# GreatV/oar-ocr

Hardware: AMD Instinct MI355X
Metric: images/sec end-to-end PP-OCRv6 det+rec (higher is better)
Workload: dtype f32; 1 GPU; PP-OCRv6-tiny-class det+rec (synthetic-weight graphs: det 447089 params, rec 1135700 params, V=6906), batch=32 synthetic 960x960 pages per GPU, 40 text lines/page; timed region = u8 pages in pageable HOST memory -> oar_ocr_predict -> oar_ocr_decode -> sorted boxes + texts + scores on the host; image_batch_size=32, region_batch_size=256, parallelism=image-parallel x1

## Files before the change

oar_ocr_amd/csrc/kernels.hip:

```cpp
#include "kernels.h"

#include <hip/hip_ext.h>
#include <hip/hip_runtime.h>

#include <algorithm>
#include <cstdlib>
#include <type_traits>

#include "common.h"
#include "kernels_dev.h"

namespace oar {
namespace k {

template <int K, int SH, int S, int TW, int TH, bool GAP = false>
__global__ __launch_bounds__(256) void conv_dw_tiled_kernel(ConvP p) {
    extern __shared__ float4 dw_w[];
    const int C4 = p.Cout >> 2;
    for (int i = threadIdx.x; i < K * K * C4; i += blockDim.x) dw_w[i] = reinterpret_cast<const float4*>(p.w)[i];
    __syncthreads();
    const int wtiles = (p.Wo + TW - 1) / TW, htiles = (p.Ho + TH - 1) / TH;
    const long total = (long)p.N * htiles * wtiles * C4;
    constexpr int NCOL = (TW - 1) * S + K, NROW = (TH - 1) * SH + K;
    const long per_xcd = (total + 7) / 8;
// ... 139 lines not shown
#define DW2(KV, SHV, SWV, THV)                                                                                                                              \
    do {                                                                                                                                                    \
        if (lds > 64 * 1024) {                                                                                                                              \
            OAR_MAX_LDS_ONCE((conv_dw_tiled_kernel<KV, SHV, SWV, TW, THV>), 96 * 1024);                    \
        }                                                                                                                                                   \
        hipExtLaunchKernelGGL((conv_dw_tiled_kernel<KV, SHV, SWV, TW, THV>), g, b, lds, s, ps.start(), ps.stop(), 0, p);                                    \
    } while (0)
#define DW2G(KV, SHV, SWV, THV)                                                                                                                             \
    do {                                                                                                                                                    \
        if (lds > 64 * 1024) {                                                                                                                              \
            OAR_MAX_LDS_ONCE((conv_dw_tiled_kernel<KV, SHV, SWV, TW, THV, true>), 96 * 1024);                    \
        }                                                                                                                                                   \
        hipExtLaunchKernelGGL((conv_dw_tiled_kernel<KV, SHV, SWV, TW, THV, true>), g, b, lds, s, ps.start(), ps.stop(), 0, p);                              \
    } while (0)
#define DWG(KV, SHV, SWV)                                  \
    do {                                                   \
        if (TH == 2) DW2G(KV, SHV, SWV, 2);                \
        else DW2G(KV, SHV, SWV, 1);                        \
    } while (0)
#define DW(KV, SHV, SWV)                                   \
    do {                                                   \
        if (TH == 2) DW2(KV, SHV, SWV, 2);                 \
        else DW2(KV, SHV, SWV, 1);                         \
    } while (0)
    if (p.gap_part) {
        if (p.sh == 1 && p.sw == 1) DWG(5, 1, 1);
        else if (p.sh == 2 && p.sw == 2) DWG(5, 2, 2);
        else if (p.sh == 2 && p.sw == 1) DWG(5, 2, 1);
        else DWG(5, 1, 2);
    } else
    if (fits && sq && p.kh == 3 && p.sh == 1 && p.sw == 1) DW(3, 1, 1);
    else if (fits && sq && p.kh == 3 && p.sh == 2 && p.sw == 2) DW(3, 2, 2);
    else if (fits && sq && p.kh == 3 && p.sh == 2 && p.sw == 1) DW(3, 2, 1);
    else if (fits && sq && p.kh == 3 && p.sh == 1 && p.sw == 2) DW(3, 1, 2);
    else if (fits && sq && p.kh == 5 && p.sh == 1 && p.sw == 1) DW(5, 1, 1);
    else if (fits && sq && p.kh == 5 && p.sh == 2 && p.sw == 2) DW(5, 2, 2);
    else if (fits && sq && p.kh == 5 && p.sh == 2 && p.sw == 1) DW(5, 2, 1);
    else if (fits && sq && p.kh == 5 && p.sh == 1 && p.sw == 2) DW(5, 1, 2);
    else hipExtLaunchKernelGGL(conv_dw_kernel, dim3(grid_for(total)), b, 0, s, ps.start(), ps.stop(), 0, p);
#undef DW2
#undef DW
#undef DW2G
#undef DWG
}

__global__ __launch_bounds__(256) void conv_smallcin_kernel(ConvP p) {
    __shared__ float ws[128 * 16];
    const int K = p.kh * p.kw * p.Cin;
    const int co0 = blockIdx.y * 16;
    for (int i = threadIdx.x; i < K * 16; i += 256) {
        int k = i >> 4, c = i & 15;
        ws[i] = (co0 + c < p.Cout) ? p.w[(long)k * p.Cout + co0 + c] : 0.f;
    }
    __syncthreads();
    const long total = (long)p.N * p.Ho * p.Wo;
    for (long pix = (long)blockIdx.x * blockDim.x + threadIdx.x; pix < total; pix += (long)gridDim.x * blockDim.x) {
        int ow = (int)(pix % p.Wo); long t = pix / p.Wo;
        int oh = (int)(t % p.Ho); long n = t / p.Ho;
        float acc[16];
#pragma unroll
        for (int c = 0; c < 16; ++c) acc[c] = (p.bias && co0 + c < p.Cout) ? p.bias[co0 + c] : 0.f;
        const float* xb = p.x + n * (long)p.H * p.W * p.Cin;
        for (int a = 0; a < p.kh; ++a) {
            int ih = oh * p.sh - p.pt + a * p.dh;
            if (ih < 0 || ih >= p.H) continue;
            for (int b = 0; b < p.kw; ++b) {
                int iw = ow * p.sw - p.pl + b * p.dw;
                if (iw < 0 || iw >= p.W) continue;
                const float* xp = xb + ((long)ih * p.W + iw) * p.Cin;
                const float* wp = ws + (a * p.kw + b) * p.Cin * 16;
                for (int ci = 0; ci < p.Cin; ++ci) {
                    float xv = xp[ci];
#pragma unroll
                    for (int c = 0; c < 16; ++c) acc[c] = fmaf(xv, wp[ci * 16 + c], acc[c]);
                }
            }
        }
        float* o = p.y + pix * p.y_ld + co0;
        const bool vec = (co0 + 16 <= p.Cout) && ((p.y_ld & 3) == 0);
#pragma unroll
        for (int c = 0; c < 16; ++c) {
            if (p.residual && co0 + c < p.Cout) acc[c] += p.residual[pix * p.y_ld + co0 + c];
            acc[c] = apply_act(acc[c], p.act.kind, p.act.alpha, p.act.beta);
        }
        if (vec) {
#pragma unroll
            for (int q = 0; q < 4; ++q) *reinterpret_cast<float4*>(o + q * 4) = make_float4(acc[q * 4], acc[q * 4 + 1], acc[q * 4 + 2], acc[q * 4 + 3]);
        } else {
            for (int c = 0; c < 16 && co0 + c < p.Cout; ++c) o[c] = acc[c];
        }
    }
}

typedef const __attribute__((address_space(4))) float sfloat;
template <bool CRNN, bool K3, bool SW>
__global__ __launch_bounds__(256) void conv_smallcin_u8_kernel(ConvP p, StemU8 st) {
    __shared__ float ws[SW ? 1 : 128 * 16];
    __shared__ float lut[CRNN ? 256 : 1];
    __shared__ float ot[4 * 64 * 17];
    const int K = p.kh * p.kw * 3;
    const int co0 = blockIdx.y * 16;
    if (!SW)
        for (int i = threadIdx.x; i < K * 16; i += 256) {
            int k = i >> 4, c = i & 15;
            ws[i] = (co0 + c < p.Cout) ? p.w[(long)k * p.Cout + co0 + c] : 0.f;
        }
    sfloat* wsc = (sfloat*)(uintptr_t)(p.w + co0);
    if (CRNN) lut[threadIdx.x] = ((float)threadIdx.x / 255.0f - 0.5f) / 0.5f;
    __syncthreads();
    const long per_image = (long)p.Ho * p.Wo;
    const float a0 = st.alpha[0], a1 = st.alpha[1], a2 = st.alpha[2], b0 = st.beta[0], b1 = st.beta[1], b2 = st.beta[2];
    const int s0 = st.src[0], s1 = st.src[1], s2 = st.src[2];
    const int n = blockIdx.z;
    const uint8_t* __restrict__ pg = CRNN ? st.dev[n].ptr : st.pages[n];
    const int img_w = CRNN ? st.dev[n].w : p.W;
    for (long pix = (long)blockIdx.x * blockDim.x + threadIdx.x; pix - (threadIdx.x & 63) < per_image; pix += (long)gridDim.x * blockDim.x) {
        const bool live = pix < per_image;
        const long pixc = live ? pix : per_image - 1;
        const int ow = (int)(pixc % p.Wo), oh = (int)(pixc / p.Wo);
        float acc[16];
#pragma unroll
        for (int c = 0; c < 16; ++c) acc[c] = (p.bias && co0 + c < p.Cout) ? p.bias[co0 + c] : 0.f;
        auto tap = [&](int a, int b, int kw) __attribute__((always_inline)) {
            const int ih = oh * p.sh - p.pt + a * p.dh, iw = ow * p.sw - p.pl + b * p.dw;
            if (ih < 0 || ih >= p.H || iw < 0 || iw >= img_w) return;
            const uint8_t* xp = pg + ((long)ih * img_w + iw) * 3;
            float x0, x1, x2;
            if (CRNN) {
                x0 = lut[xp[s0]]; x1 = lut[xp[s1]]; x2 = lut[xp[s2]];
            } else {
                const float t0 = (float)xp[s0] * a0, t1 = (float)xp[s1] * a1, t2 = (float)xp[s2] * a2;
                x0 = t0 + b0; x1 = t1 + b1; x2 = t2 + b2;
            }
            if (SW) {
                sfloat* wp = wsc + (long)(a * kw + b) * 3 * p.Cout;
#pragma unroll
                for (int c = 0; c < 16; ++c) acc[c] = fmaf(x0, wp[c], acc[c]);
#pragma unroll
                for (int c = 0; c < 16; ++c) acc[c] = fmaf(x1, wp[p.Cout + c], acc[c]);
#pragma unroll
                for (int c = 0; c < 16; ++c) acc[c] = fmaf(x2, wp[2 * p.Cout + c], acc[c]);
            } else {
                const float* wp = ws + (a * kw + b) * 3 * 16;
#pragma unroll
                for (int c = 0; c < 16; ++c) acc[c] = fmaf(x0, wp[c], acc[c]);
#pragma unroll
                for (int c = 0; c < 16; ++c) acc[c] = fmaf(x1, wp[16 + c], acc[c]);
#pragma unroll
                for (int c = 0; c < 16; ++c) acc[c] = fmaf(x2, wp[32 + c], acc[c]);
            }
        };
        if (K3) {
#pragma unroll
            for (int a = 0; a < 3; ++a)
#pragma unroll
                for (int b = 0; b < 3; ++b) tap(a, b, 3);
        } else {
            for (int a = 0; a < p.kh; ++a)
                for (int b = 0; b < p.kw; ++b) tap(a, b, p.kw);
        }
        const long opix = (long)n * per_image + pixc;
        float* o = p.y + opix * p.y_ld + co0;
        const bool vec = (co0 + 16 <= p.Cout) && ((p.y_ld & 3) == 0);
#pragma unroll
        for (int c = 0; c < 16; ++c) {
            if (p.residual && co0 + c < p.Cout) acc[c] += p.residual[opix * p.y_ld + co0 + c];
            acc[c] = apply_act(acc[c], p.act.kind, p.act.alpha, p.act.beta);
        }
        if (vec) {
            float* slab = ot + (threadIdx.x >> 6) * (64 * 17);
            const int lane = threadIdx.x & 63;
#pragma unroll
            for (int c = 0; c < 16; ++c) slab[lane * 17 + c] = acc[c];
            __builtin_amdgcn_wave_barrier();
            const long pix_w0 = pix - lane;
            float* ow_ = p.y + ((long)n * per_image + pix_w0) * p.y_ld + co0;
#pragma unroll
            for (int j = 0; j < 4; ++j) {
                const int e = j * 64 + lane, px = e >> 2, qd = e & 3;
                if (pix_w0 + px < per_image) {
                    const float* sp = slab + px * 17 + qd * 4;
                    *reinterpret_cast<float4*>(ow_ + (long)px * p.y_ld + qd * 4) = make_float4(sp[0], sp[1], sp[2], sp[3]);
                }
            }
            __builtin_amdgcn_wave_barrier();
        } else if (live) {
            for (int c = 0; c < 16 && co0 + c < p.Cout; ++c) o[c] = acc[c];
        }
    }
}
void conv_smallcin_u8(hipStream_t s, const ConvP& p, const StemU8& st) {
    const long per_image = (long)p.Ho * p.Wo;
    if (per_image == 0 || p.N == 0) return;
    OAR_CHECK(p.groups == 1 && p.Cin == 3 && p.kh * p.kw * 3 <= 128 && (st.dev ? p.N <= 65535 : p.N <= 32), OAR_INTERNAL, "conv_smallcin_u8: not an RGB stem");
    const double total = (double)p.N * per_image * p.Cout;
    ProfScope ps(s, "conv_smallcin", 3.0 * (double)p.N * p.H * p.W + 4.0 * total, 2.0 * total * p.kh * p.kw * 3);
    const dim3 grid(grid_for(per_image, 256, 256L * 4), (p.Cout + 15) / 16, p.N);
    const bool k3 = p.kh == 3 && p.kw == 3;
    static const bool sw_off = [] { const char* e = getenv("OAR_STEM_SW"); return e && e[0] == '0'; }();
    const bool sw = k3 && p.Cout % 16 == 0 && !sw_off;
    if (st.dev) {
        if (sw) hipLaunchKernelGGL((conv_smallcin_u8_kernel<true, true, true>), grid, dim3(256), 0, s, p, st);
        else if (k3) hipLaunchKernelGGL((conv_smallcin_u8_kernel<true, true, false>), grid, dim3(256), 0, s, p, st);
        else hipLaunchKernelGGL((conv_smallcin_u8_kernel<true, false, false>), grid, dim3(256), 0, s, p, st);
    } else {
        if (sw) hipLaunchKernelGGL((conv_smallcin_u8_kernel<false, true, true>), grid, dim3(256), 0, s, p, st);
        else if (k3) hipLaunchKernelGGL((conv_smallcin_u8_kernel<false, true, false>), grid, dim3(256), 0, s, p, st);
        else hipLaunchKernelGGL((conv_smallcin_u8_kernel<false, false, false>), grid, dim3(256), 0, s, p, st);
    }
}

__global__ __launch_bounds__(256) void conv_direct_kernel(ConvP p) {
    long total = (long)p.N * p.Ho * p.Wo * p.Cout;
    const int cpg = p.Cin / p.groups, opg = p.Cout / p.groups;
    for (long i = (long)blockIdx.x * blockDim.x + threadIdx.x; i < total; i += (long)gridDim.x * blockDim.x) {
        int co = (int)(i % p.Cout); long pix = i / p.Cout;
        int ow = (int)(pix % p.Wo); long t = pix / p.Wo;
        int oh = (int)(t % p.Ho); long n = t / p.Ho;
        int g = co / opg;
        float acc = p.bias ? p.bias[co] : 0.f;
        const float* xb = p.x + n * (long)p.H * p.W * p.Cin + (long)g * cpg;
        for (int a = 0; a < p.kh; ++a) {
            int ih = oh * p.sh - p.pt + a * p.dh;
            if (ih < 0 || ih >= p.H) continue;
            for (int b = 0; b < p.kw; ++b) {
                int iw = ow * p.sw - p.pl + b * p.dw;
                if (iw < 0 || iw >= p.W) continue;
                const float* xp = xb + ((long)ih * p.W + iw) * p.Cin;
                const float* wp = p.w + ((long)(a * p.kw + b) * cpg) * p.Cout + co;
                for (int ci = 0; ci < cpg; ++ci) acc = fmaf(xp[ci], wp[(long)ci * p.Cout], acc);
            }
        }
        long o = pix * p.y_ld + co;
        if (p.residual) acc += p.residual[o];
        p.y[o] = apply_act(acc, p.act.kind, p.act.alpha, p.act.beta);
    }
}
void conv_direct(hipStream_t s, const ConvP& p) {
    long total = (long)p.N * p.Ho * p.Wo * p.Cout;
    if (total == 0) return;
    double bytes = 4.0 * ((double)p.N * p.H * p.W * p.Cin + (double)total + (double)p.kh * p.kw * (p.Cin / p.groups) * p.Cout);
    double flops = 2.0 * (double)total * p.kh * p.kw * (p.Cin / p.groups);
    if (p.groups == 1 && p.Cin <= 4 && p.kh * p.kw * p.Cin <= 128) {
        ProfScope ps(s, "conv_smallcin", bytes, flops);
        long pixels = (long)p.N * p.Ho * p.Wo;
        hipLaunchKernelGGL(conv_smallcin_kernel, dim3(grid_for(pixels, 256, 256L * 16), (p.Cout + 15) / 16), dim3(256), 0, s, p);
        return;
    }
    ProfScope ps(s, "conv_direct", bytes, flops);
    hipLaunchKernelGGL(conv_direct_kernel, dim3(grid_for(total)), dim3(256), 0, s, p);
}

template <int C1>
__global__ __launch_bounds__(256) void convt2x2_pair_kernel(ConvT2Pair p) {
    extern __shared__ float4 cp_lds[];
    float4* w1 = cp_lds;
    float* w2 = reinterpret_cast<float*>(cp_lds + (long)p.C0 * C1);
    for (int i = threadIdx.x; i < p.C0 * C1; i += blockDim.x) w1[i] = reinterpret_cast<const float4*>(p.w1)[i];
    for (int i = threadIdx.x; i < C1 * 4 * p.C2; i += blockDim.x) w2[i] = p.w2[i];
    __syncthreads();
    const long total = (long)p.N * p.H * p.W * 4;
    const int Wo = p.W * 4, Ho = p.H * 4;
    for (long i = (long)blockIdx.x * blockDim.x + threadIdx.x; i < total; i += (long)gridDim.x * blockDim.x) {
        const int wb = (int)(i % (2 * p.W));
        const long t = i / (2 * p.W);
        const int a = (int)(t & 1);
        const long nh = t >> 1;
        const int h = (int)(nh % p.H);
        const long n = nh / p.H;
        const int w = wb >> 1, b = wb & 1, pos = a * 2 + b;
        const float* xp = p.x + ((n * p.H + h) * (long)p.W + w) * p.C0;
        float mid[C1];
#pragma unroll
        for (int c = 0; c < C1; ++c) mid[c] = p.b1 ? p.b1[c] : 0.f;
        for (int c4 = 0; c4 < p.C0; c4 += 4) {
            const float4 xv = *reinterpret_cast<const float4*>(xp + c4);
            const float xs[4] = {xv.x, xv.y, xv.z, xv.w};
#pragma unroll
            for (int e = 0; e < 4; ++e) {
                const float4* wr = w1 + ((long)(c4 + e) * 4 + pos) * (C1 / 4);
#pragma unroll
                for (int q = 0; q < C1 / 4; ++q) {
                    const float4 wv = wr[q];
                    mid[q * 4 + 0] = fmaf(xs[e], wv.x, mid[q * 4 + 0]); mid[q * 4 + 1] = fmaf(xs[e], wv.y, mid[q * 4 + 1]);
                    mid[q * 4 + 2] = fmaf(xs[e], wv.z, mid[q * 4 + 2]); mid[q * 4 + 3] = fmaf(xs[e], wv.w, mid[q * 4 + 3]);
                }
            }
        }
#pragma unroll
        for (int c = 0; c < C1; ++c) mid[c] = apply_act(mid[c], p.act1.kind, p.act1.alpha, p.act1.beta);
        const long orow = (n * Ho + 4 * h + 2 * a) * (long)Wo + 4 * w + 2 * b;
#pragma unroll
        for (int a2 = 0; a2 < 2; ++a2)
#pragma unroll
            for (int b2 = 0; b2 < 2; ++b2)
                for (int co = 0; co < p.C2; ++co) {
                    float acc = p.b2 ? p.b2[co] : 0.f;
#pragma unroll
                    for (int c = 0; c < C1; ++c) acc = fmaf(mid[c], w2[(c * 4 + a2 * 2 + b2) * p.C2 + co], acc);
                    p.y[(orow + (long)a2 * Wo + b2) * p.C2 + co] = apply_act(acc, p.act2.kind, p.act2.alpha, p.act2.beta);
                }
    }
}
bool convt2x2_pair_supported(int C0, int C1, int C2) {
    return C0 > 0 && (C0 & 3) == 0 && (C1 == 8 || C1 == 16 || C1 == 24 || C1 == 32) && C2 >= 1 && C2 <= 4 && (size_t)C0 * C1 * 16 + (size_t)C1 * 4 * C2 * 4 <= 60 * 1024;
}
void convt2x2_pair(hipStream_t s, const ConvT2Pair& p) {
    const long total = (long)p.N * p.H * p.W * 4;
    if (total == 0) return;
    OAR_CHECK(convt2x2_pair_supported(p.C0, p.C1, p.C2), OAR_INTERNAL, "convt2x2_pair: unsupported channel counts");
    const size_t lds = (size_t)p.C0 * p.C1 * 16 + (size_t)p.C1 * 4 * p.C2 * 4;
    const double px = (double)p.N * p.H * p.W;
    ProfScope ps(s, "convt_pair", 4.0 * px * (p.C0 + 16.0 * p.C2), 2.0 * px * 4.0 * ((double)p.C0 * p.C1 + 4.0 * p.C1 * p.C2));
    const dim3 grid(grid_for(total, 256, 256L * 8));
    switch (p.C1) {
        case 8: hipLaunchKernelGGL(convt2x2_pair_kernel<8>, grid, dim3(256), lds, s, p); break;
        case 16: hipLaunchKernelGGL(convt2x2_pair_kernel<16>, grid, dim3(256), lds, s, p); break;
        case 24: hipLaunchKernelGGL(convt2x2_pair_kernel<24>, grid, dim3(256), lds, s, p); break;
        default: hipLaunchKernelGGL(convt2x2_pair_kernel<32>, grid, dim3(256), lds, s, p); break;
    }
}

__global__ __launch_bounds__(256) void convt_direct_kernel(ConvP p) {
    long total = (long)p.N * p.Ho * p.Wo * p.Cout;
    for (long i = (long)blockIdx.x * blockDim.x + threadIdx.x; i < total; i += (long)gridDim.x * blockDim.x) {
        int co = (int)(i % p.Cout); long pix = i / p.Cout;
        int ow = (int)(pix % p.Wo); long t = pix / p.Wo;
        int oh = (int)(t % p.Ho); long n = t / p.Ho;
        float acc = p.bias ? p.bias[co] : 0.f;
        for (int a = 0; a < p.kh; ++a) {
            int th = oh + p.pt - a * p.dh;
            if (th < 0 || th % p.sh) continue;
            int ih = th / p.sh;
            if (ih >= p.H) continue;
            for (int b = 0; b < p.kw; ++b) {
                int tw = ow + p.pl - b * p.dw;
                if (tw < 0 || tw % p.sw) continue;
                int iw = tw / p.sw;
                if (iw >= p.W) continue;
                const float* xp = p.x + ((n * p.H + ih) * (long)p.W + iw) * p.Cin;
                const float* wp = p.w + ((long)(a * p.kw + b) * p.Cin) * p.Cout + co;
                for (int ci = 0; ci < p.Cin; ++ci) acc = fmaf(xp[ci], wp[(long)ci * p.Cout], acc);
            }
        }
        p.y[pix * p.y_ld + co] = apply_act(acc, p.act.kind, p.act.alpha, p.act.beta);
    }
}
void convt_direct(hipStream_t s, const ConvP& p) {
    long total = (long)p.N * p.Ho * p.Wo * p.Cout;
    if (total == 0) return;
    ProfScope ps(s, "convt_direct", 4.0 * ((double)p.N * p.H * p.W * p.Cin + (double)total), 2.0 * (double)p.N * p.H * p.W * p.Cin * p.Cout * p.kh * p.kw);
    hipLaunchKernelGGL(convt_direct_kernel, dim3(grid_for(total)), dim3(256), 0, s, p);
}

__global__ __launch_bounds__(256) void pool2d_kernel(PoolP p) {
    long total = (long)p.N * p.Ho * p.Wo * p.C;
    for (long i = (long)blockIdx.x * blockDim.x + threadIdx.x; i < total; i += (long)gridDim.x * blockDim.x) {
        int c = (int)(i % p.C); long pix = i / p.C;
        int ow = (int)(pix % p.Wo); long t = pix / p.Wo;
        int oh = (int)(t % p.Ho); long n = t / p.Ho;
        float acc = p.is_max ? -3.402823466e38f : 0.f;
        int cnt = 0;
        for (int a = 0; a < p.kh; ++a) {
            int ih = oh * p.sh - p.pt + a;
            if (ih < 0 || ih >= p.H) continue;
            for (int b = 0; b < p.kw; ++b) {
                int iw = ow * p.sw - p.pl + b;
                if (iw < 0 || iw >= p.W) continue;
                float v = p.x[((n * p.H + ih) * (long)p.W + iw) * p.C + c];
                if (p.is_max) acc = fmaxf(acc, v); else acc += v;
                ++cnt;
            }
        }
        if (!p.is_max) {
            const int ih0 = oh * p.sh - p.pt, iw0 = ow * p.sw - p.pl;
            const int full = (min(ih0 + p.kh, p.H + p.pb) - ih0) * (min(iw0 + p.kw, p.W + p.pr) - iw0);
            acc = acc / (float)(p.count_include_pad ? (full > 0 ? full : 1) : (cnt > 0 ? cnt : 1));
        }
        p.y[i] = acc;
    }
}
void pool2d(hipStream_t s, const PoolP& p) {
    long total = (long)p.N * p.Ho * p.Wo * p.C;
    if (total == 0) return;
    ProfScope ps(s, "pool2d", 4.0 * ((double)p.N * p.H * p.W * p.C + (double)total), 0.0);
    hipLaunchKernelGGL(pool2d_kernel, dim3(grid_for(total)), dim3(256), 0, s, p);
}

__global__ __launch_bounds__(256) void global_avgpool_kernel(const float* x, float* y, int HW, int C, int splits, float div) {
    extern __shared__ float4 red[];
    const int C4 = C >> 2;
    const int parts = 256 / C4 > 0 ? 256 / C4 : 1;
    const int n = blockIdx.x / splits, sp = blockIdx.x - n * splits;
    const int per = (HW + splits - 1) / splits, p0 = sp * per, p1 = min(HW, p0 + per);
    const int c4 = threadIdx.x % C4, part = threadIdx.x / C4;
    float4 acc = make_float4(0.f, 0.f, 0.f, 0.f);
    if (part < parts) {
        const float4* xb = reinterpret_cast<const float4*>(x + (long)n * HW * C) + c4;
        int i = p0 + part;
        for (; i + 3 * parts < p1; i += 4 * parts) {
            float4 a = xb[(long)i * C4], b = xb[(long)(i + parts) * C4], c = xb[(long)(i + 2 * parts) * C4], d = xb[(long)(i + 3 * parts) * C4];
            acc.x += (a.x + b.x) + (c.x + d.x); acc.y += (a.y + b.y) + (c.y + d.y);
            acc.z += (a.z + b.z) + (c.z + d.z); acc.w += (a.w + b.w) + (c.w + d.w);
        }
        for (; i < p1; i += parts) { float4 a = xb[(long)i * C4]; acc.x += a.x; acc.y += a.y; acc.z += a.z; acc.w += a.w; }
        red[part * C4 + c4] = acc;
    }
    __syncthreads();
    if (part == 0) {
        float4 t = red[c4];
        for (int q = 1; q < parts; ++q) { float4 u = red[q * C4 + c4]; t.x += u.x; t.y += u.y; t.z += u.z; t.w += u.w; }
        reinterpret_cast<float4*>(y + (long)blockIdx.x * C)[c4] = make_float4(t.x / div, t.y / div, t.z / div, t.w / div);
    }
}
__global__ __launch_bounds__(256) void global_avgpool_scalar_kernel(const float* x, float* y, int HW, int C) {
    const int n = blockIdx.y, c = blockIdx.x * 256 + threadIdx.x;
    if (c >= C) return;
    const float* xb = x + (long)n * HW * C + c;
    float acc = 0.f;
    for (int i = 0; i < HW; ++i) acc += xb[(long)i * C];
    y[(long)n * C + c] = acc / (float)HW;
}
int global_avgpool_splits(int N, int HW, int C) {
    if ((C & 3) != 0 || C / 4 > 256 || N <= 0) return 1;
    int s = (1024 + N - 1) / N;
    s = std::min(s, std::max(HW / 256, 1));
    return std::max(1, std::min(s, 256));
}
void global_avgpool(hipStream_t s, const float* x, float* y, int N, int HW, int C, float* partial) {
    if (N == 0 || C == 0) return;
    char pname[64];
    const char* cls = "global_avgpool";
    if (Profiler::get().detail) { snprintf(pname, sizeof pname, "global_avgpool N=%d HW=%d C=%d", N, HW, C); cls = pname; }
    ProfScope ps(s, cls, 4.0 * (double)N * HW * C, 0.0);
    if ((C & 3) == 0 && C / 4 <= 256) {
        const int C4 = C / 4, parts = 256 / C4;
        const size_t lds = (size_t)parts * C4 * sizeof(float4);
        const int splits = partial ? global_avgpool_splits(N, HW, C) : 1;
        if (splits == 1) {
            hipLaunchKernelGGL(global_avgpool_kernel, dim3(N), dim3(256), lds, s, x, y, HW, C, 1, (float)HW);
        } else {
            hipLaunchKernelGGL(global_avgpool_kernel, dim3(N * splits), dim3(256), lds, s, x, partial, HW, C, splits, 1.0f);
            hipLaunchKernelGGL(global_avgpool_kernel, dim3(N), dim3(256), lds, s, (const float*)partial, y, splits, C, 1, (float)HW);
        }
    } else {
        hipLaunchKernelGGL(global_avgpool_scalar_kernel, dim3((C + 255) / 256, N), dim3(256), 0, s, x, y, HW, C);
    }
}

void global_avgpool_finish(hipStream_t s, const float* part, float* y, int N, int tiles, int C, int hw) {
    if (N == 0 || C == 0) return;
    OAR_CHECK((C & 3) == 0 && C <= 1024 && tiles > 0, OAR_INTERNAL, "global_avgpool_finish: channel count");
    ProfScope ps(s, "global_avgpool", 4.0 * ((double)N * tiles * C + (double)N * C), (double)N * tiles * C);
    const int C4 = C >> 2, parts = std::max(1, 256 / C4);
    hipLaunchKernelGGL(global_avgpool_kernel, dim3(N), dim3(256), (size_t)parts * C4 * sizeof(float4), s, part, y, tiles, C, 1, (float)hw);
}

__host__ __device__ __forceinline__ float src_coord(int o, float scale, int in, int out, int ctm) {
    switch (ctm) {
        case 0: return (float)o / scale;
        case 2: return out > 1 ? (float)o * (float)(in - 1) / (float)(out - 1) : 0.f;
        case 3: return out > 1 ? ((float)o + 0.5f) / scale - 0.5f : 0.f;
        default: return ((float)o + 0.5f) / scale - 0.5f;
    }
}
__host__ __device__ __forceinline__ int nearest_src(int o, float scale, int in, int out, int ctm, int nm) {
    const float f = src_coord(o, scale, in, out, ctm);
    float r;
    switch (nm) {
        case 0: r = floorf(f); break;
        case 3: r = ceilf(f); break;
        case 2: r = floorf(f + 0.5f); break;
        default: r = ceilf(f - 0.5f); break;
    }
    const int i = (int)r;
    return i < 0 ? 0 : i > in - 1 ? in - 1 : i;
}
int resize_nearest_index(int o, float scale, int in, int out, int ctm, int nearest_mode) { return nearest_src(o, scale, in, out, ctm, nearest_mode); }
__global__ __launch_bounds__(256) void resize_kernel(const float* x, float* y, int N, int H, int W, int C, int Ho, int Wo,
                                                     float sh, float sw, int mode, int ctm, int nm, int y_ld) {
    const int C4 = C >> 2;
    const bool vec = (C & 3) == 0 && (y_ld & 3) == 0;
    const int cw = vec ? C4 : C;
    long total = (long)N * Ho * Wo * cw;
    for (long i = (long)blockIdx.x * blockDim.x + threadIdx.x; i < total; i += (long)gridDim.x * blockDim.x) {
        int cc = (int)(i % cw); long pix = i / cw;
        int ow = (int)(pix % Wo); long t = pix / Wo;
        int oh = (int)(t % Ho); long n = t / Ho;
        float fy = src_coord(oh, sh, H, Ho, ctm), fx = src_coord(ow, sw, W, Wo, ctm);
        const float* xb = x + n * (long)H * W * C;
        if (mode == 0) {
            const int iy = nearest_src(oh, sh, H, Ho, ctm, nm), ix = nearest_src(ow, sw, W, Wo, ctm, nm);
            if (vec) *reinterpret_cast<float4*>(y + pix * y_ld + cc * 4) = *reinterpret_cast<const float4*>(xb + ((long)iy * W + ix) * C + cc * 4);
            else y[pix * y_ld + cc] = xb[((long)iy * W + ix) * C + cc];
        } else {
            fy = fminf(fmaxf(fy, 0.f), (float)(H - 1)); fx = fminf(fmaxf(fx, 0.f), (float)(W - 1));
            int y0 = (int)floorf(fy), x0 = (int)floorf(fx);
            int y1 = min(y0 + 1, H - 1), x1 = min(x0 + 1, W - 1);
            float wy = fy - (float)y0, wx = fx - (float)x0;
            int nc = vec ? 4 : 1;
            for (int q = 0; q < nc; ++q) {
                int c = vec ? cc * 4 + q : cc;
                float v00 = xb[((long)y0 * W + x0) * C + c], v01 = xb[((long)y0 * W + x1) * C + c];
                float v10 = xb[((long)y1 * W + x0) * C + c], v11 = xb[((long)y1 * W + x1) * C + c];
                float top = v00 + (v01 - v00) * wx, bot = v10 + (v11 - v10) * wx;
                y[pix * y_ld + c] = top + (bot - top) * wy;
            }
        }
    }
}
void resize(hipStream_t s, const float* x, float* y, int N, int H, int W, int C, int Ho, int Wo, float scale_h,
            float scale_w, int mode, int ctm, int nearest_mode, int y_ld) {
    long total = (long)N * Ho * Wo * C;
    if (total == 0) return;
    ProfScope ps(s, "resize", 4.0 * ((double)N * H * W * C + (double)total), 0.0);
    long work = ((C & 3) == 0 && (y_ld & 3) == 0) ? total / 4 : total;
    hipLaunchKernelGGL(resize_kernel, dim3(grid_for(work)), dim3(256), 0, s, x, y, N, H, W, C, Ho, Wo, scale_h, scale_w, mode, ctm, nearest_mode, y_ld);
}

__global__ __launch_bounds__(256) void concat_gather_kernel(ConcatGatherP p, float* __restrict__ y) {
    const int C4 = p.C >> 2;
    const long total = (long)p.N * p.Ho * p.Wo * C4;
    for (long i = (long)blockIdx.x * blockDim.x + threadIdx.x; i < total; i += (long)gridDim.x * blockDim.x) {
        const int c4 = (int)(i % C4);
        const long pix = i / C4;
        const int ow = (int)(pix % p.Wo);
        const long t = pix / p.Wo;
        const int oh = (int)(t % p.Ho);
        const long n = t / p.Ho;
        int sidx = 0;
#pragma unroll
        for (int q = 1; q < 8; ++q) if (q < p.n_src && c4 * 4 >= p.off[q]) sidx = q;
        const int cs = p.c[sidx], fh = p.fh[sidx], fw = p.fw[sidx];
        const int Hs = p.Ho / fh, Ws = p.Wo / fw;
        const float* src = p.x[sidx] + ((n * Hs + oh / fh) * (long)Ws + ow / fw) * cs + (c4 * 4 - p.off[sidx]);
        reinterpret_cast<float4*>(y)[i] = *reinterpret_cast<const float4*>(src);
    }
}
void concat_gather(hipStream_t s, const ConcatGatherP& p, float* y) {
    const long total = (long)p.N * p.Ho * p.Wo * p.C;
    if (total == 0) return;
    OAR_CHECK(p.n_src >= 1 && p.n_src <= 8 && (p.C & 3) == 0, OAR_INTERNAL, "concat_gather: sources / channels");
    double rd = 0;
    for (int i = 0; i < p.n_src; ++i) rd += (double)p.N * (p.Ho / p.fh[i]) * (p.Wo / p.fw[i]) * p.c[i];
    ProfScope ps(s, "resize", 4.0 * (rd + (double)total), 0.0);
    hipLaunchKernelGGL(concat_gather_kernel, dim3(grid_for(total / 4)), dim3(256), 0, s, p, y);
}

__global__ __launch_bounds__(256) void unary_kernel(const float* x, float* y, long n, int kind, float alpha, float beta) {
    long n4 = n >> 2;
    for (long i = (long)blockIdx.x * blockDim.x + threadIdx.x; i < n4; i += (long)gridDim.x * blockDim.x) {
        float4 v = reinterpret_cast<const float4*>(x)[i];
        v.x = apply_unary(v.x, kind, alpha, beta); v.y = apply_unary(v.y, kind, alpha, beta);
        v.z = apply_unary(v.z, kind, alpha, beta); v.w = apply_unary(v.w, kind, alpha, beta);
        reinterpret_cast<float4*>(y)[i] = v;
    }
    for (long i = n4 * 4 + (long)blockIdx.x * blockDim.x + threadIdx.x; i < n; i += (long)gridDim.x * blockDim.x)
        y[i] = apply_unary(x[i], kind, alpha, beta);
}
void unary(hipStream_t s, const float* x, float* y, int64_t n, Act act) {
    if (n == 0) return;
    ProfScope ps(s, "unary", 8.0 * (double)n, 0.0);
    hipLaunchKernelGGL(unary_kernel, dim3(grid_for(n / 4 + 1)), dim3(256), 0, s, x, y, (long)n, act.kind, act.alpha, act.beta);
}

struct BinP {
    int rank, op;
    long dims[6], sa[6], sb[6];
    int akind;
    float alpha, beta;
};
__device__ __forceinline__ float bin_op(float a, float b, int op) {
    switch (op) {
        case 0: return a + b;
        case 1: return a - b;
        case 2: return a * b;
        case 3: return a / b;
        case 5: return a > 0.f ? a : a * b;
        case 6: return fmaxf(a, b);
        case 7: return fminf(a, b);
        case 8: return a == b ? 1.0f : 0.0f;
        case 9: return a < b ? 1.0f : 0.0f;
        case 10: return a > b ? 1.0f : 0.0f;
        case 11: return (a != 0.0f && b != 0.0f) ? 1.0f : 0.0f;
        case 12: return (a != 0.0f || b != 0.0f) ? 1.0f : 0.0f;
        default: return powf(a, b);
    }
}
__global__ __launch_bounds__(256) void binary_kernel(const float* a, const float* b, float* y, long n, BinP p) {
    for (long i = (long)blockIdx.x * blockDim.x + threadIdx.x; i < n; i += (long)gridDim.x * blockDim.x) {
        long r = i, oa = 0, ob = 0;
#pragma unroll
        for (int d = 5; d >= 0; --d) {
            if (d < p.rank) {
                long q = r / p.dims[d]; long idx = r - q * p.dims[d]; r = q;
                oa += idx * p.sa[d]; ob += idx * p.sb[d];
            }
        }
        y[i] = apply_act(bin_op(a[oa], b[ob], p.op), p.akind, p.alpha, p.beta);
    }
}
__global__ __launch_bounds__(256) void binary_flat_kernel(const float* a, const float* b, float* y, long n, int op, int akind, float alpha, float beta) {
    long n4 = n >> 2;
    for (long i = (long)blockIdx.x * blockDim.x + threadIdx.x; i < n4; i += (long)gridDim.x * blockDim.x) {
        float4 u = reinterpret_cast<const float4*>(a)[i], v = reinterpret_cast<const float4*>(b)[i], o;
        o.x = apply_act(bin_op(u.x, v.x, op), akind, alpha, beta); o.y = apply_act(bin_op(u.y, v.y, op), akind, alpha, beta);
        o.z = apply_act(bin_op(u.z, v.z, op), akind, alpha, beta); o.w = apply_act(bin_op(u.w, v.w, op), akind, alpha, beta);
        reinterpret_cast<float4*>(y)[i] = o;
    }
    for (long i = n4 * 4 + (long)blockIdx.x * blockDim.x + threadIdx.x; i < n; i += (long)gridDim.x * blockDim.x)
        y[i] = apply_act(bin_op(a[i], b[i], op), akind, alpha, beta);
}
__global__ __launch_bounds__(256) void binary_chan_kernel(const float* a, const float* b, float* y, long total4, int C4, long hw, long b_nstride4, int op, int akind, float alpha, float beta) {
    for (long i = (long)blockIdx.x * blockDim.x + threadIdx.x; i < total4; i += (long)gridDim.x * blockDim.x) {
        int c4 = (int)(i % C4); long pix = i / C4; long n = pix / hw;
        float4 u = reinterpret_cast<const float4*>(a)[i], v = reinterpret_cast<const float4*>(b)[n * b_nstride4 + c4], o;
// ... 825 lines not shown
```

Measured before the change: 2496 images/sec.

## Add per-pixel fused convtranspose pair kernel reading weights through constant address space

Adds a new fused 2x2 transposed-conv pair kernel in which one thread computes all sixteen output pixels for an input pixel. The input is read once per thread, weights are read from scalar constant-address-space pointers instead of being staged in LDS, and outputs are written as float4 rows. Activation dispatch is hoisted out of the inner loops. It is enabled by default when sizes fit in 32-bit indices and pointers are 16-byte aligned. The trade-off is higher register pressure per thread and fewer threads in flight.

Result: no change. 2504 images/sec, median of 2 (+0.3%).

```diff
diff --git a/oar_ocr_amd/csrc/kernels.hip b/oar_ocr_amd/csrc/kernels.hip
--- a/oar_ocr_amd/csrc/kernels.hip
+++ b/oar_ocr_amd/csrc/kernels.hip
@@ -465,6 +465,79 @@
                 }
     }
 }
+template <int N>
+__device__ __forceinline__ void apply_act_n(float (&v)[N], const Act& a) {
+    switch (a.kind) {
+        case ACT_NONE: return;
+#define OAR_ACT_CASE(K) case K: _Pragma("unroll") for (int c = 0; c < N; ++c) v[c] = apply_act(v[c], K, a.alpha, a.beta); return;
+        OAR_ACT_CASE(ACT_RELU) OAR_ACT_CASE(ACT_HSWISH) OAR_ACT_CASE(ACT_HSIGMOID) OAR_ACT_CASE(ACT_SIGMOID) OAR_ACT_CASE(ACT_LEAKY) OAR_ACT_CASE(ACT_CLIP)
+#undef OAR_ACT_CASE
+        default:
+            for (int c = 0; c < N; ++c) v[c] = apply_act(v[c], a.kind, a.alpha, a.beta);
+    }
+}
+typedef const __attribute__((address_space(4))) float* cfloat_p;
+template <int C1, int C2>
+__global__ __launch_bounds__(256) void convt2x2_pair_px_kernel(ConvT2Pair p) {
+    const int total = p.N * p.H * p.W;
+    const int pix = blockIdx.x * 256 + threadIdx.x;
+    if (pix >= total) return;
+    const int row = pix / p.W, w = pix - row * p.W;
+    const cfloat_p w1 = (cfloat_p)(uintptr_t)p.w1, w2 = (cfloat_p)(uintptr_t)p.w2;
+    const cfloat_p bias1 = (cfloat_p)(uintptr_t)p.b1, bias2 = (cfloat_p)(uintptr_t)p.b2;
+    const float* xp = p.x + (long)pix * p.C0;
+    const int Wo = p.W * 4;
+    float* yrow = p.y + ((long)row * 4 * Wo + 4 * w) * C2;
+#pragma unroll 1
+    for (int a = 0; a < 2; ++a) {
+        float o[2][4 * C2];
+#pragma unroll
+        for (int b = 0; b < 2; ++b) {
+            const int pos = a * 2 + b;
+            float mid[C1];
+#pragma unroll
+            for (int c = 0; c < C1; ++c) mid[c] = p.b1 ? bias1[c] : 0.f;
+            for (int c4 = 0; c4 < p.C0; c4 += 4) {
+                const float4 xv = *reinterpret_cast<const float4*>(xp + c4);
+                const float xs[4] = {xv.x, xv.y, xv.z, xv.w};
+#pragma unroll
+                for (int e = 0; e < 4; ++e) {
+                    const cfloat_p wr = w1 + ((c4 + e) * 4 + pos) * C1;
+#pragma unroll
+                    for (int c = 0; c < C1; ++c) mid[c] = fmaf(xs[e], wr[c], mid[c]);
+                }
+            }
+            apply_act_n(mid, p.act1);
+#pragma unroll
+            for (int a2 = 0; a2 < 2; ++a2)
+#pragma unroll
+                for (int b2 = 0; b2 < 2; ++b2)
+#pragma unroll
+                    for (int co = 0; co < C2; ++co) {
+                        float acc = p.b2 ? bias2[co] : 0.f;
+#pragma unroll
+                        for (int c = 0; c < C1; ++c) acc = fmaf(mid[c], w2[(c * 4 + a2 * 2 + b2) * C2 + co], acc);
+                        o[a2][(b * 2 + b2) * C2 + co] = acc;
+                    }
+        }
+        apply_act_n(o[0], p.act2); apply_act_n(o[1], p.act2);
+#pragma unroll
+        for (int a2 = 0; a2 < 2; ++a2) {
+            float4* dst = reinterpret_cast<float4*>(yrow + (long)(2 * a + a2) * Wo * C2);
+#pragma unroll
+            for (int q = 0; q < C2; ++q) dst[q] = make_float4(o[a2][q * 4], o[a2][q * 4 + 1], o[a2][q * 4 + 2], o[a2][q * 4 + 3]);
+        }
+    }
+}
+template <int C1>
+static void convt2x2_pair_px_launch(hipStream_t s, const ConvT2Pair& p, dim3 grid) {
+    switch (p.C2) {
+        case 1: hipLaunchKernelGGL((convt2x2_pair_px_kernel<C1, 1>), grid, dim3(256), 0, s, p); break;
+        case 2: hipLaunchKernelGGL((convt2x2_pair_px_kernel<C1, 2>), grid, dim3(256), 0, s, p); break;
+        case 3: hipLaunchKernelGGL((convt2x2_pair_px_kernel<C1, 3>), grid, dim3(256), 0, s, p); break;
+        default: hipLaunchKernelGGL((convt2x2_pair_px_kernel<C1, 4>), grid, dim3(256), 0, s, p); break;
+    }
+}
 bool convt2x2_pair_supported(int C0, int C1, int C2) {
     return C0 > 0 && (C0 & 3) == 0 && (C1 == 8 || C1 == 16 || C1 == 24 || C1 == 32) && C2 >= 1 && C2 <= 4 && (size_t)C0 * C1 * 16 + (size_t)C1 * 4 * C2 * 4 <= 60 * 1024;
 }
@@ -475,6 +548,18 @@
     const size_t lds = (size_t)p.C0 * p.C1 * 16 + (size_t)p.C1 * 4 * p.C2 * 4;
     const double px = (double)p.N * p.H * p.W;
     ProfScope ps(s, "convt_pair", 4.0 * px * (p.C0 + 16.0 * p.C2), 2.0 * px * 4.0 * ((double)p.C0 * p.C1 + 4.0 * p.C1 * p.C2));
+    const char* px_env = getenv("OAR_CONVT_PAIR_PX");
+    const long pixels = total / 4;
+    if (!(px_env && px_env[0] == '0') && pixels * 16 * p.C2 < (1L << 31) && pixels * p.C0 < (1L << 31) && (((size_t)p.x | (size_t)p.y) & 15) == 0) {
+        const dim3 pgrid((unsigned)((pixels + 255) / 256));
+        switch (p.C1) {
+            case 8: convt2x2_pair_px_launch<8>(s, p, pgrid); break;
+            case 16: convt2x2_pair_px_launch<16>(s, p, pgrid); break;
+            case 24: convt2x2_pair_px_launch<24>(s, p, pgrid); break;
+            default: convt2x2_pair_px_launch<32>(s, p, pgrid); break;
+        }
+        return;
+    }
     const dim3 grid(grid_for(total, 256, 256L * 8));
     switch (p.C1) {
         case 8: hipLaunchKernelGGL(convt2x2_pair_kernel<8>, grid, dim3(256), lds, s, p); break;
```
